# facebookresearch/CODD

Measured on AMD Instinct MI355X. Metric: frames/sec full CODD forward @960x540 (whole job), higher is better.
Workload: dtype f32 (split-bf16 MFMA operands, f32 accumulate; HITNet + context network + Fusion exact f32); 1 GPU; full CODD (HITNetMF + Motion/RAFT3D iters=16 + Fusion) 960x540 padded to 960x576, max_disp=320, one video per GPU, steady-state frames (idx>=1), synthetic stereo sequence, random-init weights; conv_precision=split, hip_graph=True, frames_per_gpu=305, prewarm_frames=150, side_streams=True, library=codd_amd/csrc/libcodd_hip.so, full=False

## Files before the change

### codd_amd/_abi.py

```python
import ctypes as C
import os

from . import build as _build

c_float_p = C.POINTER(C.c_float)


class View(C.Structure):
    _fields_ = [("ptr", C.c_void_p), ("ctot", C.c_int), ("coff", C.c_int)]


class XsView(C.Structure):
    _fields_ = [("ptr", C.c_void_p), ("c8", C.c_int), ("hp", C.c_int), ("wp", C.c_int), ("bt", C.c_int),
                ("bl", C.c_int), ("o8", C.c_int), ("terms", C.c_int)]


class ConvParams(C.Structure):
    _fields_ = [
        ("in0", View), ("in1", View), ("C0", C.c_int), ("C1", C.c_int),
        ("B", C.c_int), ("Hin", C.c_int), ("Win", C.c_int),
        ("wpacked", C.c_void_p), ("bias", C.c_void_p),
        ("res1", View), ("res2", View), ("post", View),
        ("out", C.c_void_p), ("out_ctot", C.c_int), ("out_coff", C.c_int),
        ("Cout", C.c_int), ("Hout", C.c_int), ("Wout", C.c_int),
# ... 42 lines not shown
    "codd_instnorm_xs": (_i, [_p, _i, _i, _i, _i, _p, _p, _i, _i, _p, XsView, _p]),
    "codd_conv2d_pack_weights_ex": (_i, [_p, _p, _i, _i, _i, _i, _i, _i, _ll, _ll, _f, _p]),
    "codd_allpairs_corr": (_i, [_p, _p, _i, _i, _i, _i, _p, _p, _p, _p, _p, _p]),
    "codd_allpairs_corr_scratch": (_ll, [_i, _i, _i, _i]),
    "codd_avgpool2": (_i, [_p, _i, _i, _i, _p, _p]),
    "codd_induced_flow": (_i, [_p, _p, _i, _i, _i, _f, _f, _f, _f, _p, _p]),
    "codd_context_split": (_i, [_p, _i, _i, _p, _p, _p]),
    "codd_se3_identity": (_i, [_p, _ll, _p]),
    "codd_corr_lookup": (_i, [_p, _p, _p, _p, _p, _i, _i, _i, _i, _p, _p]),
    "codd_raft_geometry": (_i, [_p, _p, _p, _i, _i, _i, _f, _f, _f, _f, _p, _p, _p]),
    "codd_se3_gn_step": (_i, [_p, _p, _i, _p, _p, _p, _p, _i, _i, _i, _f, _f, _f, _f, _i, _f, _f, _p, _p]),
    "codd_se3_gn_scratch": (_ll, [_i, _i, _i, _i]),
    "codd_set_option": (_i, [_i, _i]),
    "codd_get_option": (_i, [_i]),
    "codd_se3_gn_step_heads": (_i, [_p, XsView, _p, _p, _p, _p, _i, _i, _i, _f, _f, _f, _f, _i, _f, _f, _p, _p, _p]),
    "codd_cvx_upsample": (_i, [_p, _p, _i, _i, _i, _i, _i, _p, _p]),
    "codd_cvx_upsample_se3_weight": (_i, [_p, _p, _p, _i, _i, _i, _p, _p, _p]),
    "codd_disp_to_depth": (_i, [_p, _ll, _f, _p, _p]),
    "codd_subsample": (_i, [_p, _i, _i, _i, _i, _i, _i, _p, _p]),
    "codd_splat": (_i, [_p, _p, _i, _i, _i, _i, _i, _p, _i, _p, _i, _i, _i, _i, _i, _f, _f, _f, _f, _f, _f,
                        _p, _p, _p, _p]),
    "codd_splat_scratch": (_ll, [_i, _i, _i, _f]),
    "codd_resize_bilinear": (_i, [_p, _i, _i, _i, _i, _i, _i, _i, _p, _i, _i, _i, _i, _p]),
    "codd_resize_bilinear_add": (_i, [_p, _i, _i, _i, _i, _i, _i, _i, _p, _i, _i, _i, _i, _p, _p]),
    "codd_add_relu": (_i, [_p, _p, _ll, _i, _p, _p]),
    "codd_copy_many": (_i, [_p, _p, _p, _i, _p]),
    "codd_timestamp": (_i, [_p, _p]),
    "codd_gru_gate_zr": (_i, [_p, _p, _p, _p, _p, _p, _i, _i, _p, _p, _p]),
    "codd_gru_gate_q": (_i, [_p, _p, _p, _p, _p, _p, _p, _i, _i, _p, _p]),
    "codd_gru_gate_zr_xs": (_i, [_p, _p, _p, _p, _p, _p, _i, _i, _i, _p, XsView, _p]),
# ... 95 lines not shown
```

### codd_amd/csrc/motion.hip

```cpp
#include "common.h"
#include <string.h>
#include <stdlib.h>
#include "se3.h"


#define IN_MAXPARTS 32
__global__ __launch_bounds__(256) void instnorm_stats_kernel(const float* __restrict__ x, int HW, int parts,
                                                             double* __restrict__ partial) {
  __shared__ double red[2][4];
  const int bc = blockIdx.y, part = blockIdx.x;
  const float* p = x + (size_t)bc * HW;
  const float K = p[0];
  const int tid = threadIdx.x, lane = tid & 63, wave = tid >> 6;
  const int per = (HW + parts - 1) / parts, i0 = part * per, i1 = min(HW, i0 + per);
  float s = 0.f, q = 0.f;
  for (int i = i0 + tid; i < i1; i += 256) { const float d = p[i] - K; s += d; q += d * d; }
  double sd = (double)s, qd = (double)q;
#pragma unroll
  for (int o = 32; o > 0; o >>= 1) { sd += __shfl_xor(sd, o, 64); qd += __shfl_xor(qd, o, 64); }
  if (lane == 0) { red[0][wave] = sd; red[1][wave] = qd; }
  __syncthreads();
  if (tid == 0) {
    partial[((size_t)bc * parts + part) * 2] = red[0][0] + red[0][1] + red[0][2] + red[0][3];
    partial[((size_t)bc * parts + part) * 2 + 1] = red[1][0] + red[1][1] + red[1][2] + red[1][3];
// ... 145 lines not shown
  avgpool2_kernel<<<cdiv(total, 256), 256, 0, (hipStream_t)stream>>>(in, h, w, out, total);
  CODD_LAUNCH_CHECK();
  return CODD_OK;
}

struct LookupGeom {
  const float *T, *d1, *d2;
  float fx, fy, cx, cy;
  float *xyz, *minfo;
  codd_xs_view cxs, mxs;
};
__device__ __forceinline__ void raft_geometry_pixel(const float* __restrict__ T, const float* __restrict__ d1,
                                                    const float* __restrict__ d2, int b, int pix, int h, int w,
                                                    float fx, float fy, float cx, float cy, float* __restrict__ xyz,
                                                    float* __restrict__ minfo, const codd_xs_view* mxs = nullptr);

#ifndef LOOKUP_PPW
#define LOOKUP_PPW 4
#endif
template <bool XS>
__global__ __launch_bounds__(256) void corr_lookup_kernel(const float* __restrict__ l0, const float* __restrict__ l1,
                                                          const float* __restrict__ l2, const float* __restrict__ l3,
                                                          const float* __restrict__ coords, int cstride, int h, int w,
                                                          float* __restrict__ out, const LookupGeom gm) {
  constexpr int PPW = LOOKUP_PPW, NPX = 4 * PPW;
  __shared__ float tile[49][NPX + 1];
  const int lvl = blockIdx.y, b = blockIdx.z;
  const int N = h * w;
  const int n0 = blockIdx.x * NPX;
  const int tid = threadIdx.x, lane = tid & 63, wave = tid >> 6;
// ... 9 lines not shown
    live[q] = n < N;
    const int nn = live[q] ? n : N - 1;
    float px, py;
    if (coords) {
      const float* cp = coords + ((size_t)b * N + nn) * cstride;
      px = cp[0]; py = cp[1];
    } else {
      const int yy = nn / w, xx = nn - yy * w;
      const SE3T Ti = se3_load(gm.T + ((size_t)b * N + nn) * 7);
      const V3 pp = project(se3_act(Ti, inv_project(gm.d1[(size_t)b * N + nn], xx, yy, gm.fx, gm.fy, gm.cx, gm.cy)), gm.fx,
                            gm.fy, gm.cx, gm.cy);
      px = pp.x; py = pp.y;
    }
    x0[q] = px * inv; y0[q] = py * inv;
  }
  float v[PPW], dxq[PPW], dyq[PPW];
#pragma unroll
  for (int q = 0; q < PPW; ++q) {
    const int nn = live[q] ? n0 + wave * PPW + q : N - 1;
    float fx = floorf(x0[q]), fy = floorf(y0[q]);
    dxq[q] = x0[q] - fx; dyq[q] = y0[q] - fy;
    fx = fminf(fmaxf(fx, -16.f), (float)w2 + 16.f);
    fy = fminf(fmaxf(fy, -16.f), (float)h2 + 16.f);
    const int ix = (int)fx - 3 + tx, iy = (int)fy - 3 + ty;
    const bool in = (unsigned)ix < (unsigned)w2 && (unsigned)iy < (unsigned)h2 && x0[q] == x0[q] && y0[q] == y0[q];
    const float t = vol[(size_t)nn * h2 * w2 + (size_t)(in ? iy : 0) * w2 + (in ? ix : 0)];
    v[q] = in ? t : 0.f;
  }
#pragma unroll
  for (int q = 0; q < PPW; ++q) {
    const int pi = wave * PPW + q;
    const float dx = dxq[q], dy = dyq[q];
    const float vx = __shfl_down(v[q], 1, 64), vy = __shfl_down(v[q], 8, 64), vxy = __shfl_down(v[q], 9, 64);
    if (live[q] && tx < 7 && ty < 7) {
      const float r = ((1.f - dx) * (1.f - dy)) * v[q] + (dx * (1.f - dy)) * vx + ((1.f - dx) * dy) * vy + (dx * dy) * vxy;
      tile[tx * 7 + ty][pi] = r;
    }
  }
  if (!coords && lvl == 0 && tid < NPX && n0 + tid < N)
    raft_geometry_pixel(gm.T, gm.d1, gm.d2, b, n0 + tid, h, w, gm.fx, gm.fy, gm.cx, gm.cy, gm.xyz, gm.minfo,
                        XS ? &gm.mxs : nullptr);
  __syncthreads();
  if (XS) {
    const codd_xs_view& d = gm.cxs;
    const int c0 = lvl * 49, c1 = c0 + 49;
    const int of = (c0 + 7) >> 3, ol = c1 >> 3;
    for (int e = tid; e < (ol - of) * NPX; e += 256) {
      const int o = of + e / NPX, pi = e % NPX, n = n0 + pi;
      if (n >= N) continue;
      float v[8];
#pragma unroll
      for (int i = 0; i < 8; ++i) v[i] = tile[o * 8 + i - c0][pi];
// ... 49 lines not shown
                                            float fx, float fy, float cx, float cy, float* xyz, codd_xs_view minfo_xs,
                                            codd_xs_view corr_xs, void* stream) {
  if (!T || !depth1 || !depth2 || !lvl0 || !lvl1 || !lvl2 || !lvl3 || !xyz || !xs_view_ok(minfo_xs, 9, h, w) ||
      !xs_view_ok(corr_xs, 196, h, w))
    return CODD_EINVAL;
  LookupGeom gm = {T, depth1, depth2, fx, fy, cx, cy, xyz, nullptr, corr_xs, minfo_xs};
  dim3 grid(cdiv(h * w, 4 * LOOKUP_PPW), 4, B);
  corr_lookup_kernel<true><<<grid, 256, 0, (hipStream_t)stream>>>(lvl0, lvl1, lvl2, lvl3, nullptr, 0, h, w, nullptr, gm);
  CODD_LAUNCH_CHECK();
  return CODD_OK;
}


__device__ __forceinline__ float clamp50(float v) { return v != v ? v : fminf(fmaxf(v, -50.f), 50.f); }

__device__ __forceinline__ void raft_geometry_pixel(const float* __restrict__ T, const float* __restrict__ d1,
                                                    const float* __restrict__ d2, int b, int pix, int h, int w,
                                                    float fx, float fy, float cx, float cy, float* __restrict__ xyz,
                                                    float* __restrict__ minfo, const codd_xs_view* mxs) {
  const int N = h * w, n = b * N + pix, y = pix / w, x = pix - y * w;
  const SE3T Ti = se3_load(T + (size_t)n * 7);
  const V3 X1 = se3_act(Ti, inv_project(d1[n], x, y, fx, fy, cx, cy));
  const V3 p = project(X1, fx, fy, cx, cy);
  xyz[(size_t)n * 3] = p.x; xyz[(size_t)n * 3 + 1] = p.y; xyz[(size_t)n * 3 + 2] = p.z;
  float zinv = 0.f;
  if (p.x == p.x && p.y == p.y) {
    float fx0 = floorf(p.x), fy0 = floorf(p.y);
    const float ax = p.x - fx0, ay = p.y - fy0;
    fx0 = fminf(fmaxf(fx0, -4.f), (float)w + 4.f);
    fy0 = fminf(fmaxf(fy0, -4.f), (float)h + 4.f);
    const int ix = (int)fx0, iy = (int)fy0;
    const float* dp = d2 + (size_t)b * N;
    auto tap = [&](int xx, int yy) -> float {
      return ((unsigned)xx < (unsigned)w && (unsigned)yy < (unsigned)h) ? 1.f / dp[yy * w + xx] : 0.f;
    };
    zinv = (1.f - ax) * (1.f - ay) * tap(ix, iy) + ax * (1.f - ay) * tap(ix + 1, iy) +
// ... 7 lines not shown
                         10.f * phi.x, 10.f * phi.y, 10.f * phi.z, 10.f * (zinv - p.z)};
  if (mxs) {
    float v0[8], v1[8];
#pragma unroll
    for (int c = 0; c < 8; ++c) { v0[c] = clamp50(vals[c]); v1[c] = 0.f; }
    v1[0] = clamp50(vals[8]);
    xs_store8(*mxs, b, 0, y, x, v0);
    xs_store8(*mxs, b, 1, y, x, v1);
    return;
  }
  float* mp = minfo + (size_t)b * 9 * N + pix;
#pragma unroll
  for (int c = 0; c < 9; ++c) mp[(size_t)c * N] = clamp50(vals[c]);
}

__global__ void raft_geometry_kernel(const float* __restrict__ T, const float* __restrict__ d1,
                                     const float* __restrict__ d2, int B, int h, int w, float fx, float fy, float cx,
                                     float cy, float* __restrict__ xyz, float* __restrict__ minfo) {
  const int n = blockIdx.x * blockDim.x + threadIdx.x;
  const int N = h * w;
  if (n >= B * N) return;
  raft_geometry_pixel(T, d1, d2, n / N, n % N, h, w, fx, fy, cx, cy, xyz, minfo);
}

extern "C" int codd_raft_geometry(const float* T, const float* depth1, const float* depth2, int B, int h, int w,
                                  float fx, float fy, float cx, float cy, float* xyz, float* minfo, void* stream) {
  if (!T || !depth1 || !depth2 || !xyz || !minfo) return CODD_EINVAL;
  raft_geometry_kernel<<<cdiv((long long)B * h * w, 128), 128, 0, (hipStream_t)stream>>>(T, depth1, depth2, B, h, w, fx,
                                                                                        fy, cx, cy, xyz, minfo);
  CODD_LAUNCH_CHECK();
// ... 15 lines not shown
  for (int k = 0; k < 9; ++k) gp[2 * k] = v[k];
  gp[20] = 0.f; gp[22] = 0.f;
  if (xj == w - 1 && !(xj & 1)) {
#pragma unroll
    for (int k = 0; k < 12; ++k) gp[2 * k + 1] = 0.f;
  }
}
static __device__ __forceinline__ void gn_geo2_store_a2(float* __restrict__ geo2, int b, int h, int w, int yj, int xj, float a2) {
  if (!geo2) return;
  const int wp2 = (w + 1) >> 1;
  geo2[(((size_t)b * h + yj) * wp2 + (xj >> 1)) * 24 + (xj & 1) + 18] = a2;
}
__global__ void se3_gn_prep_kernel(const float* __restrict__ ae, int ae_c, const float* __restrict__ xyz,
                                   const float* __restrict__ delta, const float* __restrict__ wgt,
                                   const float* __restrict__ d1, int h, int w, float fx, float fy, float cx, float cy,
                                   float* __restrict__ jd, int* __restrict__ cnt, int ntiles, float* __restrict__ geo2) {
  const int N = h * w;
  const int j = blockIdx.x * blockDim.x + threadIdx.x, b = blockIdx.y;
  if (j < ntiles) cnt[b * ntiles + j] = 0;
  if (j >= N) return;
  const int yj = j / w, xj = j - yj * w;
  const float* aeb = ae + (size_t)b * ae_c * N;
  float* rp = jd + ((size_t)b * N + j) * GN_JS;
  float av[GN_AE];
#pragma unroll
  for (int c = 0; c < GN_AE; ++c) av[c] = aeb[(size_t)min(c, ae_c - 1) * N + j];
  float a2 = 0.f;
#pragma unroll
  for (int c = 0; c < GN_AE; ++c) {
    const float v = av[c] * (c < ae_c ? 0.125f : 0.f);
    rp[c] = v;
    a2 += v * v;
  }
  const V3 X = inv_project(d1[(size_t)b * N + j], xj, yj, fx, fy, cx, cy);
// ... 1 lines not shown
  const float* db = delta + (size_t)b * 3 * N + j;
  const float* wb = wgt + (size_t)b * 3 * N + j;
  rp[32] = X.x; rp[33] = X.y; rp[34] = X.z;
  rp[35] = xb[0] + db[0]; rp[36] = xb[1] + db[N]; rp[37] = xb[2] + db[2 * N];
  rp[38] = wb[0]; rp[39] = wb[N]; rp[40] = wb[2 * N];
  rp[41] = a2; rp[42] = 0.f; rp[43] = 0.f;
  gn_geo2_store(geo2, b, h, w, yj, xj, X, rp[35], rp[36], rp[37], rp[38], rp[39], rp[40], fx, fy, cx, cy);
  gn_geo2_store_a2(geo2, b, h, w, yj, xj, a2);
}

__global__ __launch_bounds__(128) void gn_heads_prep_kernel(const codd_xs_view hs, const uint4* __restrict__ Wp,
                                                          const float* __restrict__ bias,
                                                          const float* __restrict__ xyz, const float* __restrict__ d1,
                                                          int h, int w, float fx, float fy, float cx, float cy,
                                                          float* __restrict__ jd, float* __restrict__ wout,
                                                          int* __restrict__ cnt, int ntiles, float* __restrict__ geo2) {
  const int N = h * w;
  const int lane = threadIdx.x & 63, px = lane & 15, g = lane >> 4, b = blockIdx.y;
  const int role = __builtin_amdgcn_readfirstlane(threadIdx.x >> 6);
  if (threadIdx.x == 0)
    for (int i = blockIdx.x; i < ntiles; i += gridDim.x) cnt[b * ntiles + i] = 0;
  const int n = blockIdx.x * 16 + px;
  const bool ok = n < N;
  const int j = ok ? n : N - 1;
  const int yj = j / w, xj = j - yj * w;
  const size_t per = (size_t)hs.c8 * hs.hp * hs.wp, ostride = (size_t)hs.hp * hs.wp;
  const bool three = CODD_TERMS_PLANES(hs.terms) == 2, f16 = CODD_TERMS_IS_F16(hs.terms);
  const uint4* src = (const uint4*)hs.ptr + (size_t)b * (three ? 2 : 1) * per +
                     ((size_t)(hs.o8 + g) * hs.hp + (yj + hs.bt)) * hs.wp + (xj + hs.bl);
  const uint4* wl = Wp + lane;
  f32x4 acc[3];
#pragma unroll
  for (int t = 0; t < 3; ++t) acc[t] = f32x4{0.f, 0.f, 0.f, 0.f};
  uint4 xh[2][8], xl[2][8], wh[2][16], wlo[2][16];
#define HEADS_LOAD(P, BUF)                                                                              \
  {                                                                                                     \
// ... 335 lines not shown
  float* pp = part + (((size_t)b * ntiles + tile) * gmax + g) * 27 * 64 + lane;
  __syncthreads();
#pragma unroll
  for (int w_ = 0; w_ < GN_WAVES; ++w_) {
    if (wave == w_) {
#pragma unroll
      for (int k = 0; k < 27; ++k) red[k][lane] = w_ == 0 ? Hs[k] : red[k][lane] + Hs[k];
    }
    __syncthreads();
  }
  for (int k = wave; k < 27; k += GN_WAVES) pp[k * 64] = red[k][lane];
}


static __device__ __forceinline__ void gn_solve_tile(float* __restrict__ T, const float (*sums)[64], int lane, int b,
                                                     int tx0, int ty0, int h, int w, float lm, float ep) {
  const int xi = tx0 + (lane & 7), yi = ty0 + (lane >> 3);
  if (xi >= w || yi >= h) return;
  const int N = h * w, i = yi * w + xi;
  float Hf[21], bf[6];
#pragma unroll
  for (int k = 0; k < 27; ++k) {
    const float s = sums[k][lane];
    if (k < 21) Hf[k] = s; else bf[k - 21] = s;
  }
  double L[6][6];
  {
    int k = 0;
#pragma unroll
    for (int p = 0; p < 6; ++p)
#pragma unroll
// ... 18 lines not shown
  double yv[6], xv[6];
#pragma unroll
  for (int p = 0; p < 6; ++p) {
    double s = (double)bf[p];
#pragma unroll
    for (int r = 0; r < p; ++r) s -= L[p][r] * yv[r];
    yv[p] = s / L[p][p];
  }
#pragma unroll
  for (int p = 5; p >= 0; --p) {
    double s = yv[p];
#pragma unroll
    for (int r = p + 1; r < 6; ++r) s -= L[r][p] * xv[r];
    xv[p] = s / L[p][p];
  }
  if (ok) {
    float* tp = T + ((size_t)b * N + i) * 7;
    const SE3T Ti = se3_load(tp);
    const SE3T dT = se3_exp(V3{(float)xv[0], (float)xv[1], (float)xv[2]}, V3{(float)xv[3], (float)xv[4], (float)xv[5]});
    se3_store(tp, se3_compose(dT, Ti));
  }
}

__global__ __launch_bounds__(64 * GN_SOLVE_WAVES) void se3_gn_solve_kernel(
    float* __restrict__ T, const float* __restrict__ part, int h, int w, int radius, int tiles_x, int ntiles, int q4,
    int gmax, float lm, float ep) {
  __shared__ float sums[27][64];
  const int lane = threadIdx.x & 63, wave = threadIdx.x >> 6;
  const int tile = blockIdx.x, b = blockIdx.y;
  const int tx0 = (tile % tiles_x) * 8, ty0 = (tile / tiles_x) * 8;
  {
    const int ylo = max(ty0 - radius, 0), yhi = min(ty0 + 7 + radius, h - 1);
    const int xlo = max(tx0 - radius, 0), xhi = min(tx0 + 7 + radius, w - 1);
    const int G = gn_groups((yhi - ylo + 1) * (xhi - xlo + 1), q4, gmax);
    const float* p = part + (((size_t)b * ntiles + tile) * gmax) * 27 * 64 + lane;
// ... 2 lines not shown
      int g = 0;
      for (; g + 4 <= G; g += 4) {
        const float v0 = p[((size_t)g * 27 + k) * 64], v1 = p[((size_t)(g + 1) * 27 + k) * 64];
        const float v2 = p[((size_t)(g + 2) * 27 + k) * 64], v3 = p[((size_t)(g + 3) * 27 + k) * 64];
        s = (((s + v0) + v1) + v2) + v3;
      }
      for (; g < G; ++g) s += p[((size_t)g * 27 + k) * 64];
      sums[k][lane] = s;
    }
  }
  __syncthreads();
  if (wave != 0) return;
  gn_solve_tile(T, sums, lane, b, tx0, ty0, h, w, lm, ep);
}

static inline int gn_q4() {
  const int q = codd_opt(CODD_OPT_GN_Q4);
  return q < 16 ? 16 : q;
}
static inline int gn_gmax(int radius) {
  const int NC = 8 + 2 * radius;
  return gn_groups(NC * NC, gn_q4(), 1 << 20);
}

static inline size_t gn_geo2_offset(int B, int h, int w, int radius) {
  const int ntiles = cdiv(w, 8) * cdiv(h, 8);
  const size_t n = (size_t)B * ntiles * gn_gmax(radius) * 27 * 64 + (size_t)B * h * w * GN_JS + (size_t)B * ntiles;
  return (n + 3) & ~(size_t)3;
}
extern "C" long long codd_se3_gn_scratch(int B, int h, int w, int radius) {
  return (long long)gn_geo2_offset(B, h, w, radius) + ((long long)B * h * ((w + 1) / 2) + 2) * GN_G2;
}
static inline int* gn_counters(float* Hb, int B, int h, int w, int radius) {
  const int ntiles = cdiv(w, 8) * cdiv(h, 8);
  return (int*)(Hb + (size_t)B * ntiles * gn_gmax(radius) * 27 * 64 + (size_t)B * h * w * GN_JS);
}

static int gn_build_solve(float* T, int B, int h, int w, float fx, float fy, float cx, float cy, int radius, float lm,
                          float ep, float* Hb, hipStream_t s) {
  const int tiles_x = cdiv(w, 8), ntiles = tiles_x * cdiv(h, 8);
  const int q4 = gn_q4(), gmax = gn_gmax(radius);
  float* part = Hb;
  const float* jd = Hb + (size_t)B * ntiles * gmax * 27 * 64;
  if (codd_opt(CODD_OPT_GN_BUILDER) == 3)
    se3_gn_build3_kernel<<<dim3(ntiles, gmax, B), 64 * GN_WAVES, 0, s>>>(T, jd, Hb + gn_geo2_offset(B, h, w, radius), h, w, fx, fy,
                                                                        cx, cy, radius, tiles_x, ntiles, q4, gmax, part);
  else
    se3_gn_build5_kernel<<<dim3(ntiles, gmax, B), 64 * GN_WAVES, 0, s>>>(T, jd, Hb + gn_geo2_offset(B, h, w, radius), h, w, fx, fy,
                                                                        cx, cy, radius, tiles_x, ntiles, q4, gmax, part);
  CODD_LAUNCH_CHECK();
  se3_gn_solve_kernel<<<dim3(ntiles, B), 64 * GN_SOLVE_WAVES, 0, s>>>(T, part, h, w, radius, tiles_x, ntiles, q4, gmax, lm, ep);
  CODD_LAUNCH_CHECK();
  return CODD_OK;
}

extern "C" int codd_se3_gn_step(float* T, const float* ae, int ae_c, const float* xyz, const float* delta,
                                const float* weight, const float* depth1, int B, int h, int w, float fx, float fy,
                                float cx, float cy, int radius, float lm, float ep, float* Hb, void* stream) {
  if (!T || !ae || !xyz || !delta || !weight || !depth1 || !Hb || ae_c < 1 || ae_c > GN_AE || radius < 0)
    return CODD_EINVAL;
  const int ntiles = cdiv(w, 8) * cdiv(h, 8);
  float* jd = Hb + (size_t)B * ntiles * gn_gmax(radius) * 27 * 64;
  hipStream_t s = (hipStream_t)stream;
  se3_gn_prep_kernel<<<dim3(cdiv(h * w, 128), B), 128, 0, s>>>(ae, ae_c, xyz, delta, weight, depth1, h, w, fx, fy, cx,
                                                             cy, jd, gn_counters(Hb, B, h, w, radius), ntiles,
                                                             Hb + gn_geo2_offset(B, h, w, radius));
  CODD_LAUNCH_CHECK();
  return gn_build_solve(T, B, h, w, fx, fy, cx, cy, radius, lm, ep, Hb, s);
}

extern "C" int codd_se3_gn_step_heads(float* T, codd_xs_view hidden, const void* head_w, const float* head_b,
                                      const float* xyz, const float* depth1, int B, int h, int w, float fx, float fy,
                                      float cx, float cy, int radius, float lm, float ep, float* weight_out, float* Hb,
                                      void* stream) {
  if (!T || !head_w || ((uintptr_t)head_w & 15) || !head_b || !xyz || !depth1 || !weight_out || !Hb || radius < 0 ||
      !xs_view_ok(hidden, 768, h, w))
    return CODD_EINVAL;
  const int ntiles = cdiv(w, 8) * cdiv(h, 8);
  float* jd = Hb + (size_t)B * ntiles * gn_gmax(radius) * 27 * 64;
  hipStream_t s = (hipStream_t)stream;
  gn_heads_prep_kernel<<<dim3(cdiv(h * w, 16), B), 128, 0, s>>>(hidden, (const uint4*)head_w, head_b, xyz, depth1, h, w, fx, fy, cx, cy,
                                                               jd, weight_out, gn_counters(Hb, B, h, w, radius), ntiles,
                                                               Hb + gn_geo2_offset(B, h, w, radius));
  CODD_LAUNCH_CHECK();
  return gn_build_solve(T, B, h, w, fx, fy, cx, cy, radius, lm, ep, Hb, s);
}

template <int MODE, int DIM>
__global__ __launch_bounds__(256) void cvx_upsample_kernel(const float* __restrict__ data,
                                                           const float* __restrict__ mask, int h, int w,
                                                           float* __restrict__ out) {
  const int x = blockIdx.x * 64 + (threadIdx.x & 63);
  const int wave = (threadIdx.x >> 6) + 4 * (blockIdx.z & 3);
  const int y = blockIdx.y, b = blockIdx.z >> 2;
  if (x >= w) return;
  const int N = h * w;
  constexpr int D = (MODE == 1) ? 6 : DIM;
  float nb[9][D];
#pragma unroll
  for (int k = 0; k < 9; ++k) {
// ... 552 lines not shown
```

### codd_amd/motion.py

```python

import numpy as np
import torch
import torch.nn as nn

from . import ops
from .hrnet import ResizeConcatConv
from .ops import Slice
from .registry import MODELS, build_backbone, build_loss, register
from .stereo import cv, packed

BF_DEFAULT = 1050 * 0.2
MERGE_ENC_HEADS = True
FUSE_NORM_RECORDS = True
FUSE_GATES = True
FNET_CORESIDENT = False
PRELOOP_SIDE = True
ENC_CORESIDENT = 1
LOOP_FORK_ENC = True
LOOP_FORK_ZR = True

def packed_cat(mods):
    ver = tuple((m.weight.data_ptr(), m.weight._version, m.bias._version) for m in mods)
    cache = mods[0].__dict__.setdefault("_codd_packed_cat", {})
    key = tuple(id(m) for m in mods)
# ... 385 lines not shown
        T = pl["T"] if pl is not None else ops.se3_identity(B, h, w, image_curr.device)
        pre = pend.pop("pyr", None)
        fmap_curr = self._join("fmap", dev)
        if fmap_curr is None:
            fmap_curr = self.fnet(image_curr)
        pyr = pre[1] if pre is not None and pre[0] is fmap_prev else ops.allpairs_corr(fmap_prev, fmap_curr)
        net, inp = (pl["net"], pl["inp"]) if pl is not None else ops.context_split(net_inp)
        if pl is not None and pl.get("depth_prev") is depth_prev:
            d1 = pl["d1"]
        else:
            d1 = ops.subsample(depth_prev.contiguous(), 3, 3, 8)
        d2 = ops.subsample(depth_curr.contiguous(), 3, 3, 8)
        mask = weight = None
        zr = pl["zr"] if pl is not None else None
        cxs, mxs = self.update_block.input_buffers(net)
        for it in range(iters):
            xyz, minfo, corr = ops.raft_geometry_lookup(T, d1, d2, K8, pyr, minfo_xs=mxs, corr_xs=cxs)
            net, mask, ae, delta, weight, zr, hid = self.update_block.run(
                net, inp, corr, minfo, need_mask=it == iters - 1, zr=zr, prefetch_next=it < iters - 1, fuse_heads=True)
            if hid is not None:
                weight = ops.se3_gn_step_heads(T, hid, *self.update_block.head_matrix(), xyz, d1, K8, radius=32)
            else:
                ops.se3_gn_step(T, ae, xyz, delta, weight, d1, K8, radius=32)
        self.update_block._forks(dev)[0].join()
        T_up, outputs["weight"] = ops.cvx_upsample_se3_weight(T, weight.contiguous(), mask)
        outputs["Ts"] = T_up
        outputs["flow2d_est_induced"] = ops.induced_flow(T_up, depth_prev, [float(v) for v in K])
        state["raft_feat"] = fmap_curr
        ni = self._join("netinp", dev)
        state["raft_netinp"] = ni if ni is not None else self.context(image_curr)


@register
class Motion(ops.RuntimeState, nn.Module):

    def __init__(self, raft3d=None, ds_scale=4, iters=16, loss=None):
# ... 52 lines not shown
```

### codd_amd/ops.py

```python
import collections
import ctypes as C

import torch

from . import _abi
from ._abi import ACT, ConvParams, View


class RuntimeState:
    _RUNTIME_KEYS = ("_side", "_pending", "_nowait", "_fk", "_xs", "_runners", "_kside", "_h4c", "_ctx4c", "_fused_now", "_pipe")

    def __getstate__(self):
        state = self.__dict__.copy()
        for k in self._RUNTIME_KEYS:
            state.pop(k, None)
        return state


class Slice:
    __slots__ = ("buf", "coff", "c")

    def __init__(self, buf, coff=0, c=None):
        assert buf.is_contiguous() and buf.dtype == torch.float32
        self.buf, self.coff = buf, coff
# ... 1082 lines not shown
                                    scratch.data_ptr(), _stream()), "se3_gn_step")
    return T


def se3_gn_step_heads(T, hidden_xs, head_w, head_b, xyz, d1, K8, radius=32, lm=1e-4, ep=10.0):
    lib = _abi.load()
    B, h, w, _ = T.shape
    scratch = _f32(lib.codd_se3_gn_scratch(B, h, w, radius), like=T)
    wout = _f32(B, 3, h, w, like=T)
    _abi.check(lib.codd_se3_gn_step_heads(T.data_ptr(), _xs_view(hidden_xs), head_w.data_ptr(), head_b.data_ptr(),
                                          xyz.data_ptr(), d1.data_ptr(), B, h, w, *K8, radius, lm, ep, wout.data_ptr(),
                                          scratch.data_ptr(), _stream()), "se3_gn_step_heads")
    return wout


def cvx_upsample(data, mask, mode):
    lib = _abi.load()
    if mode == 2:
        B, D, h, w = data.shape
        out = _f32(B, D, 8 * h, 8 * w, like=data)
    else:
        B, h, w, D = data.shape
        out = _f32(B, 8 * h, 8 * w, D, like=data)
    _abi.check(lib.codd_cvx_upsample(data.data_ptr(), mask.data_ptr(), B, h, w, D, mode, out.data_ptr(), _stream()),
               "cvx_upsample")
    return out


def cvx_upsample_se3_weight(T, weight, mask):
    lib = _abi.load()
# ... 386 lines not shown
```

### include/codd_hip.h

```cpp
#ifndef CODD_HIP_H
#define CODD_HIP_H

#ifdef __cplusplus
extern "C" {
#endif

#define CODD_ABI_VERSION 12

#define CODD_OK 0
#define CODD_EINVAL (-1)
#define CODD_EUNSUPPORTED (-2)

enum { CODD_OPT_GN_Q4 = 0, CODD_OPT_GN_BUILDER = 1, CODD_OPT_COUNT = 2 };
int codd_set_option(int key, int value);
int codd_get_option(int key);

enum { CODD_ACT_NONE = 0, CODD_ACT_LRELU02 = 1, CODD_ACT_RELU = 2, CODD_ACT_SIGMOID = 3,
       CODD_ACT_TANH = 4, CODD_ACT_MISH = 5, CODD_ACT_RELU_CH0 = 6 };

typedef struct {
  const float* ptr;
  int ctot;
  int coff;
} codd_view;
// ... 113 lines not shown

int codd_raft_geometry(const float* T, const float* depth1, const float* depth2, int B, int h, int w,
                       float fx, float fy, float cx, float cy, float* xyz, float* minfo, void* stream);

long long codd_se3_gn_scratch(int B, int h, int w, int radius);
int codd_se3_gn_step(float* T, const float* ae, int ae_c, const float* xyz, const float* delta,
                     const float* weight, const float* depth1, int B, int h, int w,
                     float fx, float fy, float cx, float cy, int radius, float lm, float ep,
                     float* Hb, void* stream);

int codd_se3_gn_step_heads(float* T, codd_xs_view hidden, const void* head_w, const float* head_b,
                           const float* xyz, const float* depth1, int B, int h, int w, float fx, float fy,
                           float cx, float cy, int radius, float lm, float ep, float* weight_out, float* Hb,
                           void* stream);

int codd_cvx_upsample(const float* data, const float* mask, int B, int h, int w, int dim, int mode,
                      float* out, void* stream);
int codd_cvx_upsample_se3_weight(const float* T, const float* weight, const float* mask, int B, int h, int w,
                                 float* T_out, float* weight_out, void* stream);

int codd_disp_to_depth(const float* disp, long long n, float bf, float* depth, void* stream);
int codd_subsample(const float* in, int B, int H, int W, int oy, int ox, int step, float* out, void* stream);

long long codd_splat_scratch(int B, int H, int W, float radius);
int codd_splat(const float* T, const float* depth, int HT, int WT, int oy, int ox, int ds,
               const float* featA, int CA, const float* featB, int CB, int with_flow,
               int B, int H, int W, float fx, float fy, float cx, float cy, float radius,
               float bf, float* out, float* zout, int* scratch, void* stream);

int codd_induced_flow(const float* T, const float* depth, int B, int H, int W,
// ... 93 lines not shown
```

Before: 106.7 frames/s.

## Fuse SE3 Gauss-Newton solve with next iteration's geometry and correlation lookup

Splits the GN step into a build stage and a solve stage. For every iteration except the last, the per-tile 6x6 solve runs in a new kernel that also recomputes reprojection geometry and gathers all four correlation pyramid levels for the next iteration, writing straight into the split-precision input buffers. This removes a separate raft_geometry_lookup launch and the global round trip of the updated poses in each RAFT3D iteration. The counter zeroing in the prep kernels is also dropped. The cost is a larger fused kernel (9 waves, big shared tiles) with less occupancy, and the geometry work is now serialized behind the solve inside one block.

Measured after the change: 107.0 frames/s, median of 2. No clear change (+0.3%).

```diff
diff --git a/codd_amd/_abi.py b/codd_amd/_abi.py
--- a/codd_amd/_abi.py
+++ b/codd_amd/_abi.py
@@ -80,6 +80,10 @@
     "codd_set_option": (_i, [_i, _i]),
     "codd_get_option": (_i, [_i]),
     "codd_se3_gn_step_heads": (_i, [_p, XsView, _p, _p, _p, _p, _i, _i, _i, _f, _f, _f, _f, _i, _f, _f, _p, _p, _p]),
+    "codd_se3_gn_build_heads": (_i, [_p, XsView, _p, _p, _p, _p, _i, _i, _i, _f, _f, _f, _f, _i, _p, _p, _ll, _p]),
+    "codd_se3_gn_solve": (_i, [_p, _i, _i, _i, _i, _f, _f, _p, _ll, _p]),
+    "codd_se3_gn_solve_lookup_xs": (_i, [_p, _p, _ll, _p, _p, _p, _p, _p, _p, _i, _i, _i, _f, _f, _f, _f, _i, _f, _f, _i, _p,
+                                         XsView, XsView, _p]),
     "codd_cvx_upsample": (_i, [_p, _p, _i, _i, _i, _i, _i, _p, _p]),
     "codd_cvx_upsample_se3_weight": (_i, [_p, _p, _p, _i, _i, _i, _p, _p, _p]),
     "codd_disp_to_depth": (_i, [_p, _ll, _f, _p, _p]),
diff --git a/codd_amd/csrc/motion.hip b/codd_amd/csrc/motion.hip
--- a/codd_amd/csrc/motion.hip
+++ b/codd_amd/csrc/motion.hip
@@ -183,6 +183,22 @@
                                                     const float* __restrict__ d2, int b, int pix, int h, int w,
                                                     float fx, float fy, float cx, float cy, float* __restrict__ xyz,
                                                     float* __restrict__ minfo, const codd_xs_view* mxs = nullptr);
+
+__device__ __forceinline__ float lookup_frac(float x0) { return x0 - floorf(x0); }
+__device__ __forceinline__ float lookup_gather(const float* __restrict__ slice, float x0, float y0, int h2, int w2,
+                                               int tx, int ty) {
+  float fx = floorf(x0), fy = floorf(y0);
+  fx = fminf(fmaxf(fx, -16.f), (float)w2 + 16.f);
+  fy = fminf(fmaxf(fy, -16.f), (float)h2 + 16.f);
+  const int ix = (int)fx - 3 + tx, iy = (int)fy - 3 + ty;
+  const bool in = (unsigned)ix < (unsigned)w2 && (unsigned)iy < (unsigned)h2 && x0 == x0 && y0 == y0;
+  const float g = slice[(size_t)(in ? iy : 0) * w2 + (in ? ix : 0)];
+  return in ? g : 0.f;
+}
+__device__ __forceinline__ float lookup_blend(float v, float dx, float dy) {
+  const float vx = __shfl_down(v, 1, 64), vy = __shfl_down(v, 8, 64), vxy = __shfl_down(v, 9, 64);
+  return ((1.f - dx) * (1.f - dy)) * v + (dx * (1.f - dy)) * vx + ((1.f - dx) * dy) * vy + (dx * dy) * vxy;
+}
 
 #ifndef LOOKUP_PPW
 #define LOOKUP_PPW 4
@@ -222,28 +238,17 @@
     }
     x0[q] = px * inv; y0[q] = py * inv;
   }
-  float v[PPW], dxq[PPW], dyq[PPW];
+  float v[PPW];
 #pragma unroll
   for (int q = 0; q < PPW; ++q) {
     const int nn = live[q] ? n0 + wave * PPW + q : N - 1;
-    float fx = floorf(x0[q]), fy = floorf(y0[q]);
-    dxq[q] = x0[q] - fx; dyq[q] = y0[q] - fy;
-    fx = fminf(fmaxf(fx, -16.f), (float)w2 + 16.f);
-    fy = fminf(fmaxf(fy, -16.f), (float)h2 + 16.f);
-    const int ix = (int)fx - 3 + tx, iy = (int)fy - 3 + ty;
-    const bool in = (unsigned)ix < (unsigned)w2 && (unsigned)iy < (unsigned)h2 && x0[q] == x0[q] && y0[q] == y0[q];
-    const float t = vol[(size_t)nn * h2 * w2 + (size_t)(in ? iy : 0) * w2 + (in ? ix : 0)];
-    v[q] = in ? t : 0.f;
+    v[q] = lookup_gather(vol + (size_t)nn * h2 * w2, x0[q], y0[q], h2, w2, tx, ty);
   }
 #pragma unroll
   for (int q = 0; q < PPW; ++q) {
     const int pi = wave * PPW + q;
-    const float dx = dxq[q], dy = dyq[q];
-    const float vx = __shfl_down(v[q], 1, 64), vy = __shfl_down(v[q], 8, 64), vxy = __shfl_down(v[q], 9, 64);
-    if (live[q] && tx < 7 && ty < 7) {
-      const float r = ((1.f - dx) * (1.f - dy)) * v[q] + (dx * (1.f - dy)) * vx + ((1.f - dx) * dy) * vy + (dx * dy) * vxy;
-      tile[tx * 7 + ty][pi] = r;
-    }
+    const float r = lookup_blend(v[q], lookup_frac(x0[q]), lookup_frac(y0[q]));
+    if (live[q] && tx < 7 && ty < 7) tile[tx * 7 + ty][pi] = r;
   }
   if (!coords && lvl == 0 && tid < NPX && n0 + tid < N)
     raft_geometry_pixel(gm.T, gm.d1, gm.d2, b, n0 + tid, h, w, gm.fx, gm.fy, gm.cx, gm.cy, gm.xyz, gm.minfo,
@@ -323,12 +328,11 @@
 
 __device__ __forceinline__ float clamp50(float v) { return v != v ? v : fminf(fmaxf(v, -50.f), 50.f); }
 
-__device__ __forceinline__ void raft_geometry_pixel(const float* __restrict__ T, const float* __restrict__ d1,
-                                                    const float* __restrict__ d2, int b, int pix, int h, int w,
-                                                    float fx, float fy, float cx, float cy, float* __restrict__ xyz,
-                                                    float* __restrict__ minfo, const codd_xs_view* mxs) {
+__device__ __forceinline__ void raft_geometry_pixel_pose(const SE3T Ti, const float* __restrict__ d1,
+                                                         const float* __restrict__ d2, int b, int pix, int h, int w,
+                                                         float fx, float fy, float cx, float cy, float* __restrict__ xyz,
+                                                         float* __restrict__ minfo, const codd_xs_view* mxs) {
   const int N = h * w, n = b * N + pix, y = pix / w, x = pix - y * w;
-  const SE3T Ti = se3_load(T + (size_t)n * 7);
   const V3 X1 = se3_act(Ti, inv_project(d1[n], x, y, fx, fy, cx, cy));
   const V3 p = project(X1, fx, fy, cx, cy);
   xyz[(size_t)n * 3] = p.x; xyz[(size_t)n * 3 + 1] = p.y; xyz[(size_t)n * 3 + 2] = p.z;
@@ -366,6 +370,13 @@
   for (int c = 0; c < 9; ++c) mp[(size_t)c * N] = clamp50(vals[c]);
 }
 
+__device__ __forceinline__ void raft_geometry_pixel(const float* __restrict__ T, const float* __restrict__ d1,
+                                                    const float* __restrict__ d2, int b, int pix, int h, int w,
+                                                    float fx, float fy, float cx, float cy, float* __restrict__ xyz,
+                                                    float* __restrict__ minfo, const codd_xs_view* mxs) {
+  raft_geometry_pixel_pose(se3_load(T + ((size_t)b * h * w + pix) * 7), d1, d2, b, pix, h, w, fx, fy, cx, cy, xyz, minfo, mxs);
+}
+
 __global__ void raft_geometry_kernel(const float* __restrict__ T, const float* __restrict__ d1,
                                      const float* __restrict__ d2, int B, int h, int w, float fx, float fy, float cx,
                                      float cy, float* __restrict__ xyz, float* __restrict__ minfo) {
@@ -411,10 +422,9 @@
 __global__ void se3_gn_prep_kernel(const float* __restrict__ ae, int ae_c, const float* __restrict__ xyz,
                                    const float* __restrict__ delta, const float* __restrict__ wgt,
                                    const float* __restrict__ d1, int h, int w, float fx, float fy, float cx, float cy,
-                                   float* __restrict__ jd, int* __restrict__ cnt, int ntiles, float* __restrict__ geo2) {
+                                   float* __restrict__ jd, float* __restrict__ geo2) {
   const int N = h * w;
   const int j = blockIdx.x * blockDim.x + threadIdx.x, b = blockIdx.y;
-  if (j < ntiles) cnt[b * ntiles + j] = 0;
   if (j >= N) return;
   const int yj = j / w, xj = j - yj * w;
   const float* aeb = ae + (size_t)b * ae_c * N;
@@ -446,12 +456,10 @@
                                                           const float* __restrict__ xyz, const float* __restrict__ d1,
                                                           int h, int w, float fx, float fy, float cx, float cy,
                                                           float* __restrict__ jd, float* __restrict__ wout,
-                                                          int* __restrict__ cnt, int ntiles, float* __restrict__ geo2) {
+                                                          float* __restrict__ geo2) {
   const int N = h * w;
   const int lane = threadIdx.x & 63, px = lane & 15, g = lane >> 4, b = blockIdx.y;
   const int role = __builtin_amdgcn_readfirstlane(threadIdx.x >> 6);
-  if (threadIdx.x == 0)
-    for (int i = blockIdx.x; i < ntiles; i += gridDim.x) cnt[b * ntiles + i] = 0;
   const int n = blockIdx.x * 16 + px;
   const bool ok = n < N;
   const int j = ok ? n : N - 1;
@@ -817,7 +825,8 @@
 
 
 static __device__ __forceinline__ void gn_solve_tile(float* __restrict__ T, const float (*sums)[64], int lane, int b,
-                                                     int tx0, int ty0, int h, int w, float lm, float ep) {
+                                                     int tx0, int ty0, int h, int w, float lm, float ep,
+                                                     float* __restrict__ tl = nullptr) {
   const int xi = tx0 + (lane & 7), yi = ty0 + (lane >> 3);
   if (xi >= w || yi >= h) return;
   const int N = h * w, i = yi * w + xi;
@@ -866,11 +875,15 @@
     for (int r = p + 1; r < 6; ++r) s -= L[r][p] * xv[r];
     xv[p] = s / L[p][p];
   }
+  float* tp = T + ((size_t)b * N + i) * 7;
   if (ok) {
-    float* tp = T + ((size_t)b * N + i) * 7;
     const SE3T Ti = se3_load(tp);
     const SE3T dT = se3_exp(V3{(float)xv[0], (float)xv[1], (float)xv[2]}, V3{(float)xv[3], (float)xv[4], (float)xv[5]});
-    se3_store(tp, se3_compose(dT, Ti));
+    const SE3T Tn = se3_compose(dT, Ti);
+    se3_store(tp, Tn);
+    if (tl) se3_store(tl + lane * 7, Tn);
+  } else if (tl) {
+    se3_store(tl + lane * 7, se3_load(tp));
   }
 }
 
@@ -903,42 +916,174 @@
   gn_solve_tile(T, sums, lane, b, tx0, ty0, h, w, lm, ep);
 }
 
-static inline int gn_q4() {
-  const int q = codd_opt(CODD_OPT_GN_Q4);
-  return q < 16 ? 16 : q;
-}
-static inline int gn_gmax(int radius) {
-  const int NC = 8 + 2 * radius;
-  return gn_groups(NC * NC, gn_q4(), 1 << 20);
-}
-
-static inline size_t gn_geo2_offset(int B, int h, int w, int radius) {
-  const int ntiles = cdiv(w, 8) * cdiv(h, 8);
-  const size_t n = (size_t)B * ntiles * gn_gmax(radius) * 27 * 64 + (size_t)B * h * w * GN_JS + (size_t)B * ntiles;
-  return (n + 3) & ~(size_t)3;
-}
-extern "C" long long codd_se3_gn_scratch(int B, int h, int w, int radius) {
-  return (long long)gn_geo2_offset(B, h, w, radius) + ((long long)B * h * ((w + 1) / 2) + 2) * GN_G2;
-}
-static inline int* gn_counters(float* Hb, int B, int h, int w, int radius) {
-  const int ntiles = cdiv(w, 8) * cdiv(h, 8);
-  return (int*)(Hb + (size_t)B * ntiles * gn_gmax(radius) * 27 * 64 + (size_t)B * h * w * GN_JS);
-}
-
-static int gn_build_solve(float* T, int B, int h, int w, float fx, float fy, float cx, float cy, int radius, float lm,
-                          float ep, float* Hb, hipStream_t s) {
-  const int tiles_x = cdiv(w, 8), ntiles = tiles_x * cdiv(h, 8);
-  const int q4 = gn_q4(), gmax = gn_gmax(radius);
-  float* part = Hb;
-  const float* jd = Hb + (size_t)B * ntiles * gmax * 27 * 64;
+#define GNL_LW 8
+#define GNL_PPW (64 / GNL_LW)
+#define GNL_WAVES (GNL_LW + 1)
+#define GNL_GC 28
+static_assert(27 % GNL_WAVES == 0, "every wave of the fused kernel reduces the same number of sums");
+
+static __device__ __forceinline__ void xs_store4(const codd_xs_view& d, int b, int oct, int y, int x, const float* v) {
+  const size_t per = (size_t)d.c8 * d.hp * d.wp;
+  const int planes = CODD_TERMS_PLANES(d.terms);
+  const bool f16 = CODD_TERMS_IS_F16(d.terms);
+  unsigned short hi[4], lo[4];
+#pragma unroll
+  for (int i = 0; i < 4; ++i) {
+    hi[i] = xs_elem16(v[i], f16);
+    lo[i] = f16 ? xs_elem16(v[i] - (float)(_Float16)v[i], true)
+                : __builtin_bit_cast(unsigned short, (__bf16)(v[i] - (float)(__bf16)v[i]));
+  }
+  uint4* dst = (uint4*)d.ptr + (size_t)b * planes * per + ((size_t)(d.o8 + oct) * d.hp + (y + d.bt)) * d.wp + (x + d.bl);
+  *(uint2*)dst = uint2{(unsigned)hi[0] | ((unsigned)hi[1] << 16), (unsigned)hi[2] | ((unsigned)hi[3] << 16)};
+  if (planes == 2)
+    *(uint2*)(dst + per) = uint2{(unsigned)lo[0] | ((unsigned)lo[1] << 16), (unsigned)lo[2] | ((unsigned)lo[3] << 16)};
+}
+
+__global__ __launch_bounds__(64 * GNL_WAVES) void se3_gn_solve_lookup_kernel(
+    float* __restrict__ T, const float* __restrict__ part, int h, int w, int radius, int tiles_x, int ntiles, int q4,
+    int gmax, float lm, float ep, int do_solve, const float* __restrict__ l0, const float* __restrict__ l1,
+    const float* __restrict__ l2, const float* __restrict__ l3, const LookupGeom gm) {
+  __shared__ float tile[196][65];
+  __shared__ float tl[64 * 7];
+  float(*sums)[64] = (float(*)[64]) & tile[0][0];
+  const int tid = threadIdx.x, lane = tid & 63;
+  const int wave = __builtin_amdgcn_readfirstlane(tid >> 6);
+  const int tilei = blockIdx.x, b = blockIdx.y;
+  const int tx0 = (tilei % tiles_x) * 8, ty0 = (tilei / tiles_x) * 8;
+  const int N = h * w;
+  float dq[GNL_PPW];
+  if (wave < GNL_LW) {
+#pragma unroll
+    for (int q = 0; q < GNL_PPW; ++q) {
+      const int p = wave * GNL_PPW + q, xx = tx0 + (p & 7), yy = ty0 + (p >> 3);
+      dq[q] = gm.d1[(size_t)b * N + (xx < w && yy < h ? yy * w + xx : N - 1)];
+    }
+  }
+  if (do_solve) {
+    const int ylo = max(ty0 - radius, 0), yhi = min(ty0 + 7 + radius, h - 1);
+    const int xlo = max(tx0 - radius, 0), xhi = min(tx0 + 7 + radius, w - 1);
+    const int G = gn_groups((yhi - ylo + 1) * (xhi - xlo + 1), q4, gmax);
+    const float* p = part + (((size_t)b * ntiles + tilei) * gmax) * 27 * 64 + lane;
+    constexpr int KW = 27 / GNL_WAVES;
+    float s[KW];
+#pragma unroll
+    for (int i = 0; i < KW; ++i) s[i] = 0.f;
+    for (int g0 = 0; g0 < G; g0 += GNL_GC) {
+      float v[KW][GNL_GC];
+#pragma unroll
+      for (int i = 0; i < KW; ++i)
+#pragma unroll
+        for (int j = 0; j < GNL_GC; ++j)
+          v[i][j] = p[((size_t)min(g0 + j, G - 1) * 27 + (wave + i * GNL_WAVES)) * 64];
+#pragma unroll
+      for (int i = 0; i < KW; ++i)
+#pragma unroll
+        for (int j = 0; j < GNL_GC; ++j) s[i] = g0 + j < G ? s[i] + v[i][j] : s[i];
+    }
+#pragma unroll
+    for (int i = 0; i < KW; ++i) sums[wave + i * GNL_WAVES][lane] = s[i];
+  }
+  __syncthreads();
+  const int xi = tx0 + (lane & 7), yi = ty0 + (lane >> 3);
+  const bool inmap = xi < w && yi < h;
+  if (wave == GNL_LW) {
+    se3_store(tl + lane * 7, SE3T{V3{0.f, 0.f, 0.f}, Q4{0.f, 0.f, 0.f, 1.f}});
+    if (do_solve) gn_solve_tile(T, sums, lane, b, tx0, ty0, h, w, lm, ep, tl);
+    else if (inmap) se3_store(tl + lane * 7, se3_load(T + ((size_t)b * N + yi * w + xi) * 7));
+  }
+  __syncthreads();
+  if (wave == GNL_LW) {
+    if (inmap)
+      raft_geometry_pixel_pose(se3_load(tl + lane * 7), gm.d1, gm.d2, b, yi * w + xi, h, w, gm.fx, gm.fy, gm.cx, gm.cy,
+                               gm.xyz, nullptr, &gm.mxs);
+  } else {
+    const int tx = lane & 7, ty = lane >> 3;
+    float px[GNL_PPW], py[GNL_PPW];
+#pragma unroll
+    for (int q = 0; q < GNL_PPW; ++q) {
+      const int p = wave * GNL_PPW + q, xx = tx0 + (p & 7), yy = ty0 + (p >> 3);
+      const SE3T Ti = se3_load(tl + p * 7);
+      const V3 pp = project(se3_act(Ti, inv_project(dq[q], xx, yy, gm.fx, gm.fy, gm.cx, gm.cy)), gm.fx, gm.fy, gm.cx, gm.cy);
+      px[q] = pp.x; py[q] = pp.y;
+    }
+    float v[4][GNL_PPW];
+#pragma unroll
+    for (int lvl = 0; lvl < 4; ++lvl) {
+      const int h2 = h >> lvl, w2 = w >> lvl;
+      const float* vol = (lvl == 0 ? l0 : lvl == 1 ? l1 : lvl == 2 ? l2 : l3) + (size_t)b * N * h2 * w2;
+      const float inv = 1.f / (float)(1 << lvl);
+#pragma unroll
+      for (int q = 0; q < GNL_PPW; ++q) {
+        const int p = wave * GNL_PPW + q, xx = tx0 + (p & 7), yy = ty0 + (p >> 3);
+        const int nn = xx < w && yy < h ? yy * w + xx : N - 1;
+        v[lvl][q] = lookup_gather(vol + (size_t)nn * h2 * w2, px[q] * inv, py[q] * inv, h2, w2, tx, ty);
+      }
+    }
+#pragma unroll
+    for (int lvl = 0; lvl < 4; ++lvl) {
+      const float inv = 1.f / (float)(1 << lvl);
+#pragma unroll
+      for (int q = 0; q < GNL_PPW; ++q) {
+        const int p = wave * GNL_PPW + q, xx = tx0 + (p & 7), yy = ty0 + (p >> 3);
+        const float r = lookup_blend(v[lvl][q], lookup_frac(px[q] * inv), lookup_frac(py[q] * inv));
+        if (xx < w && yy < h && tx < 7 && ty < 7) tile[lvl * 49 + tx * 7 + ty][p] = r;
+      }
+    }
+  }
+  __syncthreads();
+  for (int e = tid; e < 25 * 64; e += 64 * GNL_WAVES) {
+    const int o = e >> 6, p = e & 63, xx = tx0 + (p & 7), yy = ty0 + (p >> 3);
+    if (xx >= w || yy >= h) continue;
+    float vv[8];
+#pragma unroll
+    for (int i = 0; i < 8; ++i) vv[i] = o * 8 + i < 196 ? tile[o * 8 + i][p] : 0.f;
+    if (o < 24) xs_store8(gm.cxs, b, o, yy, xx, vv);
+    else xs_store4(gm.cxs, b, o, yy, xx, vv);
+  }
+}
+
+struct GnPlan {
+  int tiles_x, ntiles, q4, gmax;
+  size_t jd_off, geo2_off;
+  long long total;
+};
+static inline GnPlan gn_plan(int B, int h, int w, int radius) {
+  GnPlan p;
+  const int q = codd_opt(CODD_OPT_GN_Q4), NC = 8 + 2 * radius;
+  p.q4 = q < 16 ? 16 : q;
+  p.gmax = gn_groups(NC * NC, p.q4, 1 << 20);
+  p.tiles_x = cdiv(w, 8);
+  p.ntiles = p.tiles_x * cdiv(h, 8);
+  p.jd_off = (size_t)B * p.ntiles * p.gmax * 27 * 64;
+  p.geo2_off = (p.jd_off + (size_t)B * h * w * GN_JS + (size_t)B * p.ntiles + 3) & ~(size_t)3;
+  p.total = (long long)p.geo2_off + ((long long)B * h * ((w + 1) / 2) + 2) * GN_G2;
+  return p;
+}
+extern "C" long long codd_se3_gn_scratch(int B, int h, int w, int radius) { return gn_plan(B, h, w, radius).total; }
+
+static int gn_build(const GnPlan& pl, const float* T, int B, int h, int w, float fx, float fy, float cx, float cy,
+                    int radius, float* Hb, hipStream_t s) {
   if (codd_opt(CODD_OPT_GN_BUILDER) == 3)
-    se3_gn_build3_kernel<<<dim3(ntiles, gmax, B), 64 * GN_WAVES, 0, s>>>(T, jd, Hb + gn_geo2_offset(B, h, w, radius), h, w, fx, fy,
-                                                                        cx, cy, radius, tiles_x, ntiles, q4, gmax, part);
+    se3_gn_build3_kernel<<<dim3(pl.ntiles, pl.gmax, B), 64 * GN_WAVES, 0, s>>>(T, Hb + pl.jd_off, Hb + pl.geo2_off, h, w, fx, fy, cx, cy,
+                                                                              radius, pl.tiles_x, pl.ntiles, pl.q4, pl.gmax, Hb);
   else
-    se3_gn_build5_kernel<<<dim3(ntiles, gmax, B), 64 * GN_WAVES, 0, s>>>(T, jd, Hb + gn_geo2_offset(B, h, w, radius), h, w, fx, fy,
-                                                                        cx, cy, radius, tiles_x, ntiles, q4, gmax, part);
-  CODD_LAUNCH_CHECK();
-  se3_gn_solve_kernel<<<dim3(ntiles, B), 64 * GN_SOLVE_WAVES, 0, s>>>(T, part, h, w, radius, tiles_x, ntiles, q4, gmax, lm, ep);
+    se3_gn_build5_kernel<<<dim3(pl.ntiles, pl.gmax, B), 64 * GN_WAVES, 0, s>>>(T, Hb + pl.jd_off, Hb + pl.geo2_off, h, w, fx, fy, cx, cy,
+                                                                              radius, pl.tiles_x, pl.ntiles, pl.q4, pl.gmax, Hb);
+  CODD_LAUNCH_CHECK();
+  return CODD_OK;
+}
+static int gn_solve(const GnPlan& pl, float* T, int B, int h, int w, int radius, float lm, float ep, const float* Hb,
+                    hipStream_t s) {
+  se3_gn_solve_kernel<<<dim3(pl.ntiles, B), 64 * GN_SOLVE_WAVES, 0, s>>>(T, Hb, h, w, radius, pl.tiles_x, pl.ntiles, pl.q4,
+                                                                        pl.gmax, lm, ep);
+  CODD_LAUNCH_CHECK();
+  return CODD_OK;
+}
+static int gn_heads_prep(const GnPlan& pl, codd_xs_view hidden, const void* head_w, const float* head_b, const float* xyz,
+                         const float* depth1, int B, int h, int w, float fx, float fy, float cx, float cy,
+                         float* weight_out, float* Hb, hipStream_t s) {
+  gn_heads_prep_kernel<<<dim3(cdiv(h * w, 16), B), 128, 0, s>>>(hidden, (const uint4*)head_w, head_b, xyz, depth1, h, w, fx, fy, cx, cy,
+                                                               Hb + pl.jd_off, weight_out, Hb + pl.geo2_off);
   CODD_LAUNCH_CHECK();
   return CODD_OK;
 }
@@ -948,14 +1093,13 @@
                                 float cx, float cy, int radius, float lm, float ep, float* Hb, void* stream) {
   if (!T || !ae || !xyz || !delta || !weight || !depth1 || !Hb || ae_c < 1 || ae_c > GN_AE || radius < 0)
     return CODD_EINVAL;
-  const int ntiles = cdiv(w, 8) * cdiv(h, 8);
-  float* jd = Hb + (size_t)B * ntiles * gn_gmax(radius) * 27 * 64;
+  const GnPlan pl = gn_plan(B, h, w, radius);
   hipStream_t s = (hipStream_t)stream;
   se3_gn_prep_kernel<<<dim3(cdiv(h * w, 128), B), 128, 0, s>>>(ae, ae_c, xyz, delta, weight, depth1, h, w, fx, fy, cx,
-                                                             cy, jd, gn_counters(Hb, B, h, w, radius), ntiles,
-                                                             Hb + gn_geo2_offset(B, h, w, radius));
-  CODD_LAUNCH_CHECK();
-  return gn_build_solve(T, B, h, w, fx, fy, cx, cy, radius, lm, ep, Hb, s);
+                                                             cy, Hb + pl.jd_off, Hb + pl.geo2_off);
+  CODD_LAUNCH_CHECK();
+  const int rc = gn_build(pl, T, B, h, w, fx, fy, cx, cy, radius, Hb, s);
+  return rc != CODD_OK ? rc : gn_solve(pl, T, B, h, w, radius, lm, ep, Hb, s);
 }
 
 extern "C" int codd_se3_gn_step_heads(float* T, codd_xs_view hidden, const void* head_w, const float* head_b,
@@ -965,14 +1109,50 @@
   if (!T || !head_w || ((uintptr_t)head_w & 15) || !head_b || !xyz || !depth1 || !weight_out || !Hb || radius < 0 ||
       !xs_view_ok(hidden, 768, h, w))
     return CODD_EINVAL;
-  const int ntiles = cdiv(w, 8) * cdiv(h, 8);
-  float* jd = Hb + (size_t)B * ntiles * gn_gmax(radius) * 27 * 64;
+  const GnPlan pl = gn_plan(B, h, w, radius);
   hipStream_t s = (hipStream_t)stream;
-  gn_heads_prep_kernel<<<dim3(cdiv(h * w, 16), B), 128, 0, s>>>(hidden, (const uint4*)head_w, head_b, xyz, depth1, h, w, fx, fy, cx, cy,
-                                                               jd, weight_out, gn_counters(Hb, B, h, w, radius), ntiles,
-                                                               Hb + gn_geo2_offset(B, h, w, radius));
-  CODD_LAUNCH_CHECK();
-  return gn_build_solve(T, B, h, w, fx, fy, cx, cy, radius, lm, ep, Hb, s);
+  int rc = gn_heads_prep(pl, hidden, head_w, head_b, xyz, depth1, B, h, w, fx, fy, cx, cy, weight_out, Hb, s);
+  if (rc == CODD_OK) rc = gn_build(pl, T, B, h, w, fx, fy, cx, cy, radius, Hb, s);
+  return rc != CODD_OK ? rc : gn_solve(pl, T, B, h, w, radius, lm, ep, Hb, s);
+}
+
+extern "C" int codd_se3_gn_build_heads(const float* T, codd_xs_view hidden, const void* head_w, const float* head_b,
+                                       const float* xyz, const float* depth1, int B, int h, int w, float fx, float fy,
+                                       float cx, float cy, int radius, float* weight_out, float* Hb,
+                                       long long scratch_floats, void* stream) {
+  if (!T || !head_w || ((uintptr_t)head_w & 15) || !head_b || !xyz || !depth1 || !weight_out || !Hb || radius < 0 ||
+      B < 1 || h < 1 || w < 1 || !xs_view_ok(hidden, 768, h, w))
+    return CODD_EINVAL;
+  const GnPlan pl = gn_plan(B, h, w, radius);
+  if (scratch_floats < pl.total) return CODD_EINVAL;
+  hipStream_t s = (hipStream_t)stream;
+  const int rc = gn_heads_prep(pl, hidden, head_w, head_b, xyz, depth1, B, h, w, fx, fy, cx, cy, weight_out, Hb, s);
+  return rc != CODD_OK ? rc : gn_build(pl, T, B, h, w, fx, fy, cx, cy, radius, Hb, s);
+}
+
+extern "C" int codd_se3_gn_solve(float* T, int B, int h, int w, int radius, float lm, float ep, const float* Hb,
+                                 long long scratch_floats, void* stream) {
+  if (!T || !Hb || radius < 0 || B < 1 || h < 1 || w < 1) return CODD_EINVAL;
+  const GnPlan pl = gn_plan(B, h, w, radius);
+  if (scratch_floats < pl.total) return CODD_EINVAL;
+  return gn_solve(pl, T, B, h, w, radius, lm, ep, Hb, (hipStream_t)stream);
+}
+
+extern "C" int codd_se3_gn_solve_lookup_xs(float* T, const float* Hb, long long scratch_floats, const float* depth1,
+                                           const float* depth2, const float* lvl0, const float* lvl1, const float* lvl2,
+                                           const float* lvl3, int B, int h, int w, float fx, float fy, float cx,
+                                           float cy, int radius, float lm, float ep, int do_solve, float* xyz,
+                                           codd_xs_view minfo_xs, codd_xs_view corr_xs, void* stream) {
+  if (!T || !depth1 || !depth2 || !lvl0 || !lvl1 || !lvl2 || !lvl3 || !xyz || radius < 0 || B < 1 || h < 8 || w < 8 ||
+      !xs_view_ok(minfo_xs, 9, h, w) || !xs_view_ok(corr_xs, 196, h, w) || (do_solve && !Hb))
+    return CODD_EINVAL;
+  const GnPlan pl = gn_plan(B, h, w, radius);
+  if (do_solve && scratch_floats < pl.total) return CODD_EINVAL;
+  LookupGeom gm = {nullptr, depth1, depth2, fx, fy, cx, cy, xyz, nullptr, corr_xs, minfo_xs};
+  se3_gn_solve_lookup_kernel<<<dim3(pl.ntiles, B), 64 * GNL_WAVES, 0, (hipStream_t)stream>>>(
+      T, Hb, h, w, radius, pl.tiles_x, pl.ntiles, pl.q4, pl.gmax, lm, ep, do_solve, lvl0, lvl1, lvl2, lvl3, gm);
+  CODD_LAUNCH_CHECK();
+  return CODD_OK;
 }
 
 template <int MODE, int DIM>
diff --git a/codd_amd/motion.py b/codd_amd/motion.py
--- a/codd_amd/motion.py
+++ b/codd_amd/motion.py
@@ -423,12 +423,19 @@
         mask = weight = None
         zr = pl["zr"] if pl is not None else None
         cxs, mxs = self.update_block.input_buffers(net)
+        scratch = ops.se3_gn_scratch(T, radius=32) if cxs is not None else None
+        xyz = None
         for it in range(iters):
-            xyz, minfo, corr = ops.raft_geometry_lookup(T, d1, d2, K8, pyr, minfo_xs=mxs, corr_xs=cxs)
+            if scratch is None or it == 0:
+                xyz, minfo, corr = ops.raft_geometry_lookup(T, d1, d2, K8, pyr, minfo_xs=mxs, corr_xs=cxs)
             net, mask, ae, delta, weight, zr, hid = self.update_block.run(
                 net, inp, corr, minfo, need_mask=it == iters - 1, zr=zr, prefetch_next=it < iters - 1, fuse_heads=True)
             if hid is not None:
-                weight = ops.se3_gn_step_heads(T, hid, *self.update_block.head_matrix(), xyz, d1, K8, radius=32)
+                weight = ops.se3_gn_build_heads(T, hid, *self.update_block.head_matrix(), xyz, d1, K8, scratch, radius=32)
+                if it < iters - 1:
+                    xyz = ops.se3_gn_solve_lookup(T, scratch, d1, d2, K8, pyr, mxs, cxs, radius=32)
+                else:
+                    ops.se3_gn_solve(T, scratch, radius=32)
             else:
                 ops.se3_gn_step(T, ae, xyz, delta, weight, d1, K8, radius=32)
         self.update_block._forks(dev)[0].join()
diff --git a/codd_amd/ops.py b/codd_amd/ops.py
--- a/codd_amd/ops.py
+++ b/codd_amd/ops.py
@@ -1120,6 +1120,41 @@
     return wout
 
 
+def se3_gn_scratch(T, radius=32):
+    B, h, w, _ = T.shape
+    return _f32(_abi.load().codd_se3_gn_scratch(B, h, w, radius), like=T)
+
+
+def se3_gn_build_heads(T, hidden_xs, head_w, head_b, xyz, d1, K8, scratch, radius=32):
+    lib = _abi.load()
+    B, h, w, _ = T.shape
+    wout = _f32(B, 3, h, w, like=T)
+    _abi.check(lib.codd_se3_gn_build_heads(T.data_ptr(), _xs_view(hidden_xs), head_w.data_ptr(), head_b.data_ptr(),
+                                           xyz.data_ptr(), d1.data_ptr(), B, h, w, *K8, radius, wout.data_ptr(),
+                                           scratch.data_ptr(), scratch.numel(), _stream()), "se3_gn_build_heads")
+    return wout
+
+
+def se3_gn_solve(T, scratch, radius=32, lm=1e-4, ep=10.0):
+    B, h, w, _ = T.shape
+    _abi.check(_abi.load().codd_se3_gn_solve(T.data_ptr(), B, h, w, radius, lm, ep, scratch.data_ptr(), scratch.numel(),
+                                             _stream()), "se3_gn_solve")
+    return T
+
+
+def se3_gn_solve_lookup(T, scratch, d1, d2, K8, pyr, minfo_xs, corr_xs, radius=32, lm=1e-4, ep=10.0, do_solve=True):
+    lib = _abi.load()
+    B, h, w, _ = T.shape
+    xyz = _f32(B, h, w, 3, like=T)
+    _abi.check(lib.codd_se3_gn_solve_lookup_xs(T.data_ptr(), scratch.data_ptr() if scratch is not None else None,
+                                               scratch.numel() if scratch is not None else 0, d1.data_ptr(),
+                                               d2.data_ptr(), pyr[0].data_ptr(), pyr[1].data_ptr(), pyr[2].data_ptr(),
+                                               pyr[3].data_ptr(), B, h, w, *K8, radius, lm, ep, int(bool(do_solve)),
+                                               xyz.data_ptr(), _xs_view(minfo_xs), _xs_view(corr_xs), _stream()),
+               "se3_gn_solve_lookup_xs")
+    return xyz
+
+
 def cvx_upsample(data, mask, mode):
     lib = _abi.load()
     if mode == 2:
diff --git a/include/codd_hip.h b/include/codd_hip.h
--- a/include/codd_hip.h
+++ b/include/codd_hip.h
@@ -151,6 +151,18 @@
                            float cx, float cy, int radius, float lm, float ep, float* weight_out, float* Hb,
                            void* stream);
 
+int codd_se3_gn_build_heads(const float* T, codd_xs_view hidden, const void* head_w, const float* head_b,
+                            const float* xyz, const float* depth1, int B, int h, int w, float fx, float fy,
+                            float cx, float cy, int radius, float* weight_out, float* Hb, long long scratch_floats,
+                            void* stream);
+int codd_se3_gn_solve(float* T, int B, int h, int w, int radius, float lm, float ep, const float* Hb,
+                      long long scratch_floats, void* stream);
+int codd_se3_gn_solve_lookup_xs(float* T, const float* Hb, long long scratch_floats, const float* depth1,
+                                const float* depth2, const float* lvl0, const float* lvl1, const float* lvl2,
+                                const float* lvl3, int B, int h, int w, float fx, float fy, float cx, float cy,
+                                int radius, float lm, float ep, int do_solve, float* xyz, codd_xs_view minfo_xs,
+                                codd_xs_view corr_xs, void* stream);
+
 int codd_cvx_upsample(const float* data, const float* mask, int B, int h, int w, int dim, int mode,
                       float* out, void* stream);
 int codd_cvx_upsample_se3_weight(const float* T, const float* weight, const float* mask, int B, int h, int w,
```
